# nygenome/Lancet2

Measured on AMD Instinct MI355X. Metric: microassembly windows/sec (whole node), higher is better.
Workload: dtype u8/i32 (f64 statistics)

## Files before the change

lancet2_amd/csrc/poa.hip:

```cpp
#include <algorithm>
#include <cstdio>
#include <cstdlib>
#include <vector>

#include "ma_internal.h"

namespace ma {

namespace {

constexpr int kT = 256;
constexpr u32 kSlowCap = 256;
constexpr u32 kMaxSeq = 32;
constexpr i32 kNegInf = static_cast<i32>(0x80000000u) + 1024;
constexpr i32 M_ = 0, N_ = -6, G_ = -6, E_ = -2, Q_ = -26, C_ = -1;

constexpr u32 kTierIn = 2;

constexpr u32 RI_FAST = 1u << 11;
constexpr u32 RI_SLOWTAB = 1u << 12;
constexpr u32 RI_STORE = 1u << 13;
constexpr u32 RI_LEAN = 1u << 14;
constexpr u32 RI_SLIDE = 1u << 15;
template <int PE>
// ... 38 lines not shown
  size_t frow_cells;
  u32 full_by_worker;
  u32 band_stride;
  u16* codes;
  i32* rows;
  i32* hlast;
  u32 split;
  u32 img_words;
  u8* img;
};

extern __shared__ __attribute__((aligned(16))) unsigned char ma_lds[];
template <class T>
struct LdsArr {
  u32 off;
  __device__ __forceinline__ T& operator[](u32 i) const { return *reinterpret_cast<T*>(&ma_lds[off + i * sizeof(T)]); }
};

struct WgState {
  u32 nn, nseq, nrank, overflow;
  i32 seq_first[kMaxSeq];
  u32 mode, V, L, cw, naln, nslow;
  u32 band, band_fail;
  u32 filled;
  i32 edge_max;
  i32 edge0;
  i32 best;
  u32 best_row;
  i32 ftot[2][4][2];
  i32 fbnd[2][4][4];
  u32 wsum[4];
  i32 red_v[4];
  u32 red_r[4];
  i32 begin, prev0, lastn;
  u32 nv;
  u32 x_done, x_a, x_ns;
  u32 win_overflow;
  u32 c_cur, h_cur, pending, done;
  u32 nvars, pool, var_overflow;
  i32 xa_active[kMaxSeq], xa_alt_of[kMaxSeq];
  u32 xa_hap_pos[kMaxSeq], xa_starts[kMaxSeq], xa_rawlen[kMaxSeq], xa_grp_rep[kMaxSeq], xa_glo[kMaxSeq], xa_ghi[kMaxSeq], xa_ordg[kMaxSeq],
      xa_rank_of_grp[kMaxSeq];
};
#define ST (*reinterpret_cast<WgState*>(ma_lds))
constexpr u32 kStBytes = (sizeof(WgState) + 15u) & ~15u;

template <int PE_>
struct GLT {
  static constexpr int pe = PE_;
  u32 pn;
  LdsArr<u8> nchar, nin, nout, nal;
  LdsArr<u16> in_tail, out_head, al, rank2node, node2rank;
  u32 lab32;
  u32 out_lab_off;
  __device__ __forceinline__ u32 lab(u32 i) const {
    return lab32 ? *reinterpret_cast<u32*>(&ma_lds[out_lab_off + 4u * i]) : static_cast<u32>(*reinterpret_cast<u16*>(&ma_lds[out_lab_off + 2u * i]));
  }
  __device__ __forceinline__ void lab_set(u32 i, u32 v) const {
    if (lab32) *reinterpret_cast<u32*>(&ma_lds[out_lab_off + 4u * i]) = v;
    else *reinterpret_cast<u16*>(&ma_lds[out_lab_off + 2u * i]) = static_cast<u16>(v);
  }
  __device__ __forceinline__ void lab_or(u32 i, u32 v) const { lab_set(i, lab(i) | v); }
  __device__ __forceinline__ u32 max_seq() const { return lab32 ? 32u : 16u; }
  LdsArr<u16> npos;
  LdsArr<u32> rowinfo;
  LdsArr<u16> rowslot, rowdepth, runhead, rowj0, slowpred, aln;
  u32 aln_cap;
  LdsArr<u16> cnode, cpos, ccur;
  LdsArr<u16> stack;
  LdsArr<u8> marks, ignored;
  u32 stack_cap;
  __device__ __forceinline__ u32 ubyte(const u8* p) const { return *p; }
  __device__ __forceinline__ u32 uword(const void* p) const { return *static_cast<const u32*>(p); }
};

__host__ __device__ inline size_t poa_lds_bytes(u32 pn, u32 ml, u32 lab32, u32 pe) {
  size_t const graph = size_t(10 + pe * (lab32 ? 10 : 8)) * pn;
  size_t const s_aln = size_t(12) * (pn + 2) + 2 * pe * kSlowCap + size_t(4) * (pn + ml + 2);
  size_t const s_topo = size_t(2 * pe + 2) * pn;
  return kStBytes + graph + (s_aln > s_topo ? s_aln : s_topo) + 16;
}

constexpr size_t kPoaLdsLimit = 160 * 1024 - 256;
inline u32 poa_node_capacity(u32 max_len, u32 lab32) {
  u32 pn = max_len + std::max<u32>(256, max_len / 4);
  pn = std::min<u32>((pn + 7) & ~7u, 65000);
  while (!lab32 && poa_lds_bytes(pn, max_len, lab32, 4) > 80 * 1024 && pn > max_len + 128) pn -= 8;
  while (poa_lds_bytes(pn, max_len, lab32, 4) > 159 * 1024 && pn > max_len + 32) pn -= 8;
  return pn;
}
inline u32 poa_node_capacity_max(u32 max_len, u32 lab32, u32 pe) {
  u32 const floor_pn = (max_len + 32 + 7) & ~7u;
  if (poa_lds_bytes(floor_pn, max_len, lab32, pe) > kPoaLdsLimit) return 0;
  u32 pn = floor_pn;
  while (pn + 8 <= 65000 && poa_lds_bytes(pn + 8, max_len, lab32, pe) <= kPoaLdsLimit) pn += 8;
  return pn;
}
inline u32 poa_retry_max_hap_len(u32 lab32, u32 pe) {
  u32 l = 4096;
  while (l > 16 && poa_node_capacity_max(l, lab32, pe) == 0) --l;
  return l;
}
inline u32 poa_max_hap_len(u32 lab32) {
  auto const scan = [](u32 lab) {
    u32 l = 4096;
    while (l > 16 && poa_lds_bytes(poa_node_capacity(l, lab), l, lab, 4) > kPoaLdsLimit) --l;
    return l;
  };
  static u32 const common = scan(0u), wide = scan(1u);
  return lab32 ? wide : common;
}

template <int PE>
__device__ __forceinline__ GLT<PE> poa_carve(u32 PN, u32 ML, u32 lab32) {
  GLT<PE> g;
  g.pn = PN;
  g.lab32 = lab32;
  u32 o = kStBytes;
  g.nchar.off = o;
  g.nin.off = o + PN;
  g.nout.off = o + 2 * PN;
  g.nal.off = o + 3 * PN;
  o += 4 * PN;
  g.in_tail.off = o;
  g.out_head.off = o + 2 * PE * PN;
  g.out_lab_off = o + 4 * PE * PN;
  g.al.off = o + (lab32 ? 8 : 6) * PE * PN;
  o += (lab32 ? 10 : 8) * PE * PN;
  g.rank2node.off = o;
  g.node2rank.off = o + 2 * PN;
  g.npos.off = o + 4 * PN;
  o += 6 * PN;
  u32 const S = o;
  g.rowinfo.off = S;
  g.rowslot.off = S + 4 * (PN + 2);
  g.rowdepth.off = S + 6 * (PN + 2);
  g.runhead.off = S + 8 * (PN + 2);
  g.rowj0.off = S + 10 * (PN + 2);
  g.slowpred.off = S + 12 * (PN + 2);
  g.aln.off = S + 12 * (PN + 2) + 2 * PE * kSlowCap;
  g.aln_cap = PN + ML + 2;
  g.cnode.off = S;
  g.cpos.off = S + 2 * (ML + 2);
  g.ccur.off = S + 4 * (ML + 2);
  g.stack.off = S;
  g.stack_cap = PE * PN;
  g.marks.off = S + 2 * PE * PN;
  g.ignored.off = S + (2 * PE + 1) * PN;
  return g;
}

__device__ __forceinline__ void lds_barrier() { asm volatile("s_waitcnt lgkmcnt(0)\n\ts_barrier" ::: "memory"); }

template <class G>
__device__ __forceinline__ i32 pg_add_node(G const& g, u8 ch, u32 pos) {
  if (ST.nn >= g.pn) {
    ST.overflow = 1;
    return 0;
  }
  u32 const id = ST.nn++;
  g.nchar[id] = ch;
  g.nin[id] = g.nout[id] = g.nal[id] = 0;
  g.npos[id] = static_cast<u16>(min(pos, 0xFFFFu));
  return static_cast<i32>(id);
}
template <class G>
__device__ __forceinline__ void pg_add_edge(G const& g, u32 tail, u32 head, u32 lab) {
  u32 const no = g.nout[tail];
  for (u32 x = 0; x < no; ++x)
    if (g.out_head[tail * G::pe + x] == head) {
      g.lab_or(tail * G::pe + x, lab);
      return;
    }
  u32 const ni = g.nin[head];
  if (no >= G::pe || ni >= G::pe) {
    atomicOr(&ST.overflow, kOvSlots);
    return;
  }
  g.out_head[tail * G::pe + no] = static_cast<u16>(head);
  g.lab_set(tail * G::pe + no, lab);
  g.nout[tail] = static_cast<u8>(no + 1);
  g.in_tail[head * G::pe + ni] = static_cast<u16>(tail);
  g.nin[head] = static_cast<u8>(ni + 1);
}
template <class G>
__device__ __forceinline__ i32 pg_add_sequence(G const& g, const u8* seq, u32 begin, u32 end) {
  if (begin >= end) return -1;
  i32 prev = -1;
  u32 const first = ST.nn;
  u32 const lab = 1u << ST.nseq;
  for (u32 i = begin; i < end; ++i) {
    i32 const cur = pg_add_node(g, seq[i], i);
    if (ST.overflow) return -1;
    if (prev >= 0) pg_add_edge(g, static_cast<u32>(prev), static_cast<u32>(cur), lab);
    prev = cur;
  }
  return static_cast<i32>(first);
}
template <class G>
__device__ __forceinline__ i32 pg_successor(G const& g, u32 node, u32 label) {
  for (int x = 0; x < g.nout[node]; ++x)
    if (g.lab(node * G::pe + x) & (1u << label)) return static_cast<i32>(g.out_head[node * G::pe + x]);
  return -1;
}
template <class G>
__device__ __forceinline__ void pg_toposort(G const& g, int lane) {
  u32 const nn = ST.nn;
  u32 nrank = 0, s = 0;
  u32 overflow = 0;
  LdsArr<u16> const stack = g.stack;
  while (s < nn && !overflow) {
    u32 const v = s + static_cast<u32>(lane);
    bool trivial = false, marked = false;
    if (v < nn) {
      marked = g.marks[v] != 0;
      if (!marked && g.nal[v] == 0) {
        u32 const ni = g.nin[v];
        bool ok = true;
        for (u32 x = 0; x < ni; ++x) ok = ok && g.in_tail[v * G::pe + x] < v;
        trivial = ok;
      }
    }
    unsigned long long const pm = __ballot(v < nn && (marked || trivial));
    u32 const run = pm == ~0ull ? 64u : static_cast<u32>(__builtin_ctzll(~pm));
    if (run > 0) {
      unsigned long long const keep = run == 64 ? ~0ull : ((1ull << run) - 1ull);
      unsigned long long const tm = __ballot(trivial) & keep;
      if (static_cast<u32>(lane) < run && trivial) {
        u32 const r = nrank + static_cast<u32>(__popcll(tm & ((1ull << lane) - 1ull)));
        g.rank2node[r] = static_cast<u16>(v);
        g.marks[v] = 2;
      }
      nrank += static_cast<u32>(__popcll(tm));
      s += run;
      continue;
    }
    if (lane == 0) {
      u32 sp = 0;
      stack[sp++] = static_cast<u16>(s);
      while (sp > 0) {
        u32 const cur = stack[sp - 1];
        bool valid = true;
        if (g.marks[cur] != 2) {
          for (int x = 0; x < g.nin[cur]; ++x) {
            u32 const t = g.in_tail[cur * G::pe + x];
            if (g.marks[t] != 2) {
              if (sp < g.stack_cap) stack[sp++] = static_cast<u16>(t); else overflow = 1;
              valid = false;
            }
          }
          if (!g.ignored[cur]) {
            for (int x = 0; x < g.nal[cur]; ++x) {
              u32 const an = g.al[cur * G::pe + x];
              if (g.marks[an] != 2) {
                if (sp < g.stack_cap) stack[sp++] = static_cast<u16>(an); else overflow = 1;
                g.ignored[an] = 1;
                valid = false;
              }
            }
          }
          if (valid) {
            g.marks[cur] = 2;
            if (!g.ignored[cur]) {
              g.rank2node[nrank++] = static_cast<u16>(cur);
              for (int x = 0; x < g.nal[cur]; ++x) g.rank2node[nrank++] = g.al[cur * G::pe + x];
            }
          } else {
            g.marks[cur] = 1;
          }
        }
        if (valid) sp--;
        if (overflow) break;
      }
    }
    nrank = __shfl(nrank, 0);
    overflow = __shfl(overflow, 0);
    s += 1;
  }
  if (lane == 0) {
    ST.nrank = nrank;
    if (overflow) ST.overflow = 1;
  }
}

__device__ __forceinline__ i32 classify_variant(const u8* r, u32 rl, const u8* a, u32 al) {
  u32 s = 0;
  while (s < rl && s < al && r[s] == a[s]) s++;
  if (s == rl && s == al) return -1;
  u32 e = 0;
  while (e < (rl - s) && e < (al - s) && r[rl - 1 - e] == a[al - 1 - e]) e++;
  u32 const rc = rl - s - e, ac = al - s - e;
  if (rc == 0 && ac > 0) return 1;
  if (rc > 0 && ac == 0) return 2;
  if (rc == 0 || ac == 0) return -1;
  if (rc != ac) return 4;
  return rc == 1 ? 0 : 3;
}
__device__ __forceinline__ i32 variant_length(const u8* r, u32 rl, const u8* a, u32 al, i32 t) {
  if (t == 0) return 1;
  i32 const R = static_cast<i32>(rl), A = static_cast<i32>(al);
  if (t == 1 || t == 2 || t == 4) return A - R;
  i32 s = 0;
  while (s < R && s < A && r[s] == a[s]) s++;
  i32 e = 0;
  while (e < (R - s) && e < (A - s) && r[R - 1 - e] == a[A - 1 - e]) e++;
  return A - s - e;
}
__device__ __forceinline__ int bytes_cmp(const u8* a, u32 al, const u8* b, u32 bl) {
  u32 const m = al < bl ? al : bl;
  for (u32 i = 0; i < m; ++i)
    if (a[i] != b[i]) return a[i] < b[i] ? -1 : 1;
  return al < bl ? -1 : (al > bl ? 1 : 0);
}

template <class G>
__device__ __forceinline__ u32 pred_row(G const& g, u32 i, u32 info, u32 x) {
  if (info & RI_FAST) return i - 1;
  if (info & RI_SLOWTAB) return g.slowpred[(G::pe <= 4 ? info >> 16 : (info >> 16) & 0xFFu) * G::pe + x];
  u32 const node = g.rank2node[i - 1];
  return static_cast<u32>(g.node2rank[g.in_tail[node * G::pe + x]]) + 1u;
// ... 1240 lines not shown
        rb[2 * static_cast<size_t>(w_stride) + c] = oo[c];
      }
      __threadfence_block();
    }
    if (L >= j0 && L < j0 + BW && static_cast<u32>(lane) == (L - j0) / CW) {
      u32 const cL = (L - j0) % CW;
      i32 v = hh[0];
#pragma unroll
      for (int c = 1; c < CW; ++c) v = (static_cast<u32>(c) == cL) ? hh[c] : v;
      hlast[i] = v;
    } else if (lane == 0 && !(L >= j0 && L < j0 + BW)) {
      hlast[i] = kNegInf;
    }
#pragma unroll
    for (int c = 0; c < CW; ++c) {
      H1[c] = hh[c];
      F1[c] = ff[c];
      O1[c] = oo[c];
    }
    __builtin_amdgcn_s_waitcnt(0);
  };

  u32 info = g.rowinfo[1];
  __builtin_amdgcn_s_waitcnt(0);
#ifdef MA_PROFILE
  unsigned long long t_lean = 0, t_gen = 0, n_gen = 0;
  unsigned long long const t_fill0 = __builtin_amdgcn_s_memtime();
#endif
  for (u32 i = 1; i <= V; ++i) {
    u32 const cur = info;
    if (i < V) info = g.rowinfo[i + 1];
#ifdef MA_PROFILE
    unsigned long long const q0 = __builtin_amdgcn_s_memtime();
#endif
    if (__builtin_expect((cur & RI_LEAN) != 0, 1)) {
      if (__builtin_expect((cur >> 16) == 0, 1)) row_lean(cur, std::false_type{});
      else row_lean(cur, std::true_type{});
    } else {
      row_gen(i, cur);
    }
#ifdef MA_PROFILE
    unsigned long long const q1 = __builtin_amdgcn_s_memtime();
    if (cur & RI_LEAN) t_lean += q1 - q0; else { t_gen += q1 - q0; n_gen++; }
#endif
    cp += BW;
  }
#ifdef MA_PROFILE
  if (lane == 0) {
    atomicAdd(&g_prof[8], t_lean);
    atomicAdd(&g_prof[9], t_gen);
    atomicAdd(&g_prof[10], n_gen);
    atomicAdd(&g_prof[11], 1ull);
    atomicAdd(&g_prof[12], static_cast<unsigned long long>(V));
    atomicAdd(&g_prof[13], __builtin_amdgcn_s_memtime() - t_fill0);
  }
#endif
  for (int off = 32; off > 0; off >>= 1) edge = max(edge, __shfl_xor(edge, off));
  if (lane == 0) *edge_out = edge;
}

struct EdgeVals {
  i32 h, f, e, o, q;
};
template <class G>
__device__ __forceinline__ EdgeVals edge_vals(G const& g, u32 i, u32 j) {
  EdgeVals v;
  if (i == 0 && j == 0) {
    v.h = v.f = v.e = v.o = v.q = 0;
  } else if (i == 0) {
    v.q = Q_ + static_cast<i32>(j - 1) * C_;
    v.e = G_ + static_cast<i32>(j - 1) * E_;
    v.h = max(v.q, v.e);
    v.f = v.o = kNegInf;
  } else {
    u32 const d = g.rowdepth[i];
    v.o = col0_o(d);
    v.f = col0_f(d);
    v.h = max(v.o, v.f);
    v.e = v.q = kNegInf;
  }
  return v;
}

template <class G>
__device__ __forceinline__ u32 poa_traceback(G const& g, const u16* codes16, size_t const plane, u32 cw, u32 V, u32 L, u32 best_row,
                             bool have_end, int lane, u32 bw) {
  const u8* const codes = reinterpret_cast<const u8*>(codes16);
  bool const band = bw != 0;
  u32 const nl = (L + cw - 1) / cw;
  bool off_band = false;
  auto code_at = [&](u32 i, u32 j) -> u32 {
    if (band) {
      u32 const j0 = g.rowj0[i];
      if (j < j0 || j >= j0 + bw) {
        off_band = true;
        return 2u;
      }
      size_t const at = static_cast<size_t>(i) * bw + (j - j0);
      u32 const a = codes[at];
      return (g.rowinfo[i] & RI_FAST) ? a : (a | (static_cast<u32>(codes[plane + at]) << 6));
    }
    size_t const at = static_cast<size_t>(i) * (nl * cw) + (j - 1);
    u32 const a = codes[at];
    return (g.rowinfo[i] & RI_FAST) ? a : (a | (static_cast<u32>(codes[plane + at]) << 6));
  };
  u32 naln = 0;
  bool overflow = false;
  auto push1 = [&](u32 node1, u32 pos1) {
    if (naln + 1 >= g.aln_cap) {
      overflow = true;
      return;
    }
    if (lane == 0) {
      g.aln[2 * naln] = static_cast<u16>(node1);
      g.aln[2 * naln + 1] = static_cast<u16>(pos1);
    }
    naln++;
  };
  u32 i = have_end ? best_row : 0u, j = have_end ? L : 0u;
  u32 prev_i = 0, prev_j = 0;
  while (!(i == 0 && j == 0) && !overflow && !__ballot(off_band)) {
    if (i >= 1 && j >= 1) {
      {
        u32 const k = static_cast<u32>(lane);
        bool ok = false;
        if (i >= k + 2 && j >= k + 1) ok = ((code_at(i - k, j - k) & 3u) == 0u) && (g.rowinfo[i - k] & RI_FAST);
        unsigned long long const m = __ballot(ok);
        u32 const run = m == ~0ull ? 64u : static_cast<u32>(__builtin_ctzll(~m));
        if (run > 0) {
          if (naln + run + 1 >= g.aln_cap) {
            overflow = true;
            break;
          }
          if (k < run) {
            g.aln[2 * (naln + k)] = static_cast<u16>(g.rank2node[i - k - 1] + 1u);
            g.aln[2 * (naln + k) + 1] = static_cast<u16>(j - k);
          }
          naln += run;
          i -= run;
          j -= run;
          prev_i = i;
          prev_j = j;
          continue;
        }
      }
      u32 const cd = code_at(i, j);
      u32 const info = g.rowinfo[i];
      u32 const np = ri_np<G::pe>(info);
      u32 const node = g.rank2node[i - 1];
      u32 const kind = cd & 3u;
      bool const ext = cd & 4u;
      constexpr u32 XB = kXB<G::pe>, XM = (1u << XB) - 1u;
      u32 const x = (cd >> 6) & XM;
      if (kind == 0) {
        prev_i = np ? pred_row(g, i, info, x) : 0u;
        prev_j = j - 1;
        push1(node + 1, j);
        i = prev_i;
        j = prev_j;
      } else if (kind == 1) {
        prev_i = np ? pred_row(g, i, info, x) : 0u;
        prev_j = j;
        push1(node + 1, 0);
        i = prev_i;
        if (ext) {
          while (!overflow && i >= 1) {
            {
              u32 const k = static_cast<u32>(lane);
              bool ok = false;
              if (i >= k + 2) ok = (code_at(i - k, j) & 16u) && (g.rowinfo[i - k] & RI_FAST);
              unsigned long long const m = __ballot(ok);
              u32 const run = m == ~0ull ? 64u : static_cast<u32>(__builtin_ctzll(~m));
              if (run > 0) {
                if (naln + run + 1 >= g.aln_cap) {
                  overflow = true;
                  break;
                }
                if (k < run) {
                  g.aln[2 * (naln + k)] = static_cast<u16>(g.rank2node[i - k - 1] + 1u);
                  g.aln[2 * (naln + k) + 1] = 0;
                }
                naln += run;
                i -= run;
                prev_i = i;
                continue;
              }
            }
            u32 const c2 = code_at(i, j);
            u32 const info2 = g.rowinfo[i];
            bool const us = c2 & 16u, uh = c2 & 32u;
            u32 const pi = (us || uh) ? pred_row(g, i, info2, (c2 >> (6 + XB)) & XM) : 0u;
            push1(g.rank2node[i - 1] + 1u, 0);
            prev_i = pi;
            i = pi;
            if (!us || i == 0) break;
          }
        }
      } else {
        prev_i = i;
        prev_j = j - 1;
        push1(0, j);
        j = prev_j;
        if (ext) {
          while (!overflow && j >= 1) {
            u32 const k = static_cast<u32>(lane);
            bool cont = false;
            if (j >= k + 1) cont = code_at(i, j - k) & 8u;
            unsigned long long const m = __ballot(cont);
            u32 const nc = m == ~0ull ? 64u : static_cast<u32>(__builtin_ctzll(~m));
            u32 const cnt = nc < 64u ? nc + 1u : 64u;
            if (naln + cnt + 1 >= g.aln_cap) {
              overflow = true;
              break;
            }
            if (k < cnt) {
              g.aln[2 * (naln + k)] = 0;
              g.aln[2 * (naln + k) + 1] = static_cast<u16>(j - k);
            }
            naln += cnt;
            j -= cnt;
            if (nc < 64u) break;
          }
        }
      }
      continue;
    }
    i32 const Hij = edge_vals(g, i, j).h;
    bool found = false, ext_left = false, ext_up = false;
    u32 const node = i ? g.rank2node[i - 1] : 0u;
    u32 const info = i ? g.rowinfo[i] : 0u;
    u32 const np = i ? (ri_np<G::pe>(info)) : 0u;
    if (i != 0) {
      for (u32 x = 0; x < (np ? np : 1u); ++x) {
        u32 const pi = np ? pred_row(g, i, info, x) : 0u;
        EdgeVals const pv = edge_vals(g, pi, j);
        bool ok = (ext_up |= (Hij == pv.f + E_));
        if (!ok) ok = Hij == pv.h + G_;
        if (!ok) ok = (ext_up |= (Hij == pv.o + C_));
        if (!ok) ok = Hij == pv.h + Q_;
        if (ok) {
          prev_i = pi;
          prev_j = j;
          found = true;
          break;
        }
      }
    }
    if (!found && j != 0) {
      EdgeVals const lv = edge_vals(g, i, j - 1);
      bool ok = (ext_left |= (Hij == lv.e + E_));
      if (!ok) ok = Hij == lv.h + G_;
      if (!ok) ok = (ext_left |= (Hij == lv.q + C_));
      if (!ok) ok = Hij == lv.h + Q_;
      if (ok) {
        prev_i = i;
        prev_j = j - 1;
        found = true;
      }
    }
    push1(i != prev_i ? node + 1 : 0u, j != prev_j ? j : 0u);
    i = prev_i;
    j = prev_j;
    if (ext_left) {
      while (!overflow) {
        push1(0, j);
        --j;
        bool const e_stop = edge_vals(g, i, j).e + E_ != edge_vals(g, i, j + 1).e;
        bool const q_stop = edge_vals(g, i, j).q + C_ != edge_vals(g, i, j + 1).q;
        if ((e_stop && q_stop) || j == 0) break;
      }
    } else if (ext_up) {
      while (!overflow && i >= 1) {
        bool stop = true;
        prev_i = 0;
        u32 const nd2 = g.rank2node[i - 1];
        u32 const info2 = g.rowinfo[i];
        u32 const np2 = ri_np<G::pe>(info2);
        EdgeVals const cv = edge_vals(g, i, j);
        for (u32 x = 0; x < np2; ++x) {
          u32 const pr = pred_row(g, i, info2, x);
          EdgeVals const pv = edge_vals(g, pr, j);
          if (cv.f == pv.f + E_ || cv.o == pv.o + C_) {
            prev_i = pr;
            stop = false;
            break;
          }
        }
        if (stop) {
          for (u32 x = 0; x < np2; ++x) {
            u32 const pr = pred_row(g, i, info2, x);
            i32 const hp2 = edge_vals(g, pr, j).h;
            if (cv.f == hp2 + G_ || cv.o == hp2 + Q_) {
              prev_i = pr;
              break;
            }
          }
        }
        push1(nd2 + 1u, 0);
        i = prev_i;
        if (stop || i == 0) break;
      }
    }
  }
  if (__ballot(off_band)) {
// ... 1345 lines not shown
  } else {
    MA_TRY_RC(launch_msa_pass(ctx, b, a, o, got[0], rounds, 0u, any_wide ? 1u : 0u, caps, cause));
    if (any_wide) MA_TRY_RC(launch_msa_pass(ctx, b, a, o, std::max(got[3], 16u), rounds, 1u, 2u, caps, cause));
  }
  if (!cause) return MA_OK;
  static RetryCaps const rcaps{{poa_retry_max_hap_len(0u, 8u), poa_retry_max_hap_len(1u, 8u), poa_retry_max_hap_len(0u, 4u), poa_retry_max_hap_len(1u, 4u)}};
  hipLaunchKernelGGL(k_poa_retry_select, dim3((n + 255) / 256), dim3(256), 0, ctx->stream, a, o.win_nvars, n, static_cast<u32>(P.max_haps),
                     static_cast<u32>(P.max_comps), cause, rcaps, all32 ? 1u : 0u, rctr);
  u32 marks[4] = {0, 0, 0, 0};
  MA_HIP(ctx, hipMemcpyAsync(marks, rctr, 16, hipMemcpyDeviceToHost, ctx->stream));
  MA_HIP(ctx, ma_stream_sync(ctx));
  ctx->poa_retry_counts[0] = marks[0];
  ctx->poa_retry_counts[1] = marks[1];
  if (marks[0] + marks[1] == 0) return MA_OK;
  u32 mx[5] = {0, 0, 0, 0, 0};
  MA_HIP(ctx, hipMemcpyAsync(mx, rctr + 4, 20, hipMemcpyDeviceToHost, ctx->stream));
  MA_HIP(ctx, ma_stream_sync(ctx));
  u32 const rrounds = std::max<u32>(1u, mx[4] + 1u);
  for (u32 k = 0; k < 4; ++k)
    if (mx[k]) MA_TRY_RC(launch_msa_pass(ctx, b, a, o, mx[k], rrounds, k & 1u, 3u + k, caps, cause));
  hipLaunchKernelGGL(k_poa_retry_count, dim3((n + 255) / 256), dim3(256), 0, ctx->stream, a, n, static_cast<const u8*>(cause), rctr);
  MA_HIP(ctx, hipMemcpyAsync(marks, rctr, 16, hipMemcpyDeviceToHost, ctx->stream));
  MA_HIP(ctx, ma_stream_sync(ctx));
  ctx->poa_retry_counts[2] = marks[2];
  ctx->poa_retry_counts[3] = marks[3];
  return MA_OK;
}
static int launch_msa_pass(ma_ctx* ctx, const DBatch& b, const ma_asm_out_t& a, const ma_var_out_t& o, u32 max_len, u32 rounds,
                           u32 const lab32, u32 const pass, const u32 (&len_caps)[3], u8* const cause) {
  int const n = b.n_windows;
  ma_params_t const& P = ctx->prm;
  PoaWs ws{};
  MA_TRY_RC(ma_dev_stats(ctx, &ws.dstats));
  ws.lab32 = lab32;
  ws.pass = pass;
  ws.cause = cause;
  bool const retry = pass >= 3;
  u32 const pe = (pass == 3 || pass == 4) ? 8u : 4u;
  ws.len_cap16 = len_caps[0];
  ws.len_cap32 = len_caps[1];
  ws.len_all32 = len_caps[2];
  max_len = std::max<u32>(max_len, 16);
  ws.max_l = max_len;
  u32 const pn = retry ? poa_node_capacity_max(max_len, lab32, pe) : poa_node_capacity(max_len, lab32);
  size_t const lds = poa_lds_bytes(pn, max_len, lab32, pe);
  if (pn == 0 || lds > kPoaLdsLimit) {
    ma_set_err(ctx, "ma_msa_batch: haplotypes too long for the LDS-resident POA graph");
    return MA_ERR_PARAM;
  }
  ws.pn = pn;
  ws.w_stride = (max_len + 7) & ~7u;
  ws.row_slots = pn / 2;
  int const band_mode = getenv("MA_POA_BAND") ? atoi(getenv("MA_POA_BAND")) : 2;
  ws.use_band = (band_mode != 0 && band_mode != 3) ? 1u : 0u;
  ws.split = band_mode >= 2 ? 1u : 0u;
  ws.no_direct = getenv("MA_POA_NO_DIRECT") ? 1u : 0u;
  ws.raw_cap = getenv("MA_POA_RAW_CAP") ? static_cast<u32>(atoi(getenv("MA_POA_RAW_CAP"))) : 0u;
  ws.lean = (getenv("MA_POA_LEAN") && atoi(getenv("MA_POA_LEAN")) == 0) ? 0u : 1u;
  {
    int const t0 = getenv("MA_POA_TIER0") ? atoi(getenv("MA_POA_TIER0")) : static_cast<int>(kTierIn);
    ws.tier0 = (t0 == 1 || t0 == 2) ? static_cast<u32>(t0) : 4u;
  }
  u32 const min_pending = getenv("MA_POA_MIN_PENDING") ? static_cast<u32>(atoi(getenv("MA_POA_MIN_PENDING"))) : 256u;
  bool const verbose = getenv("MA_VERBOSE") != nullptr;
  ws.img_words = static_cast<u32>((lds + 3) / 4);
  ws.band_stride = 256;
  ws.code_cells = (static_cast<size_t>(pn + 2) * 256 + 7) & ~size_t(7);
  if (ws.code_cells * 2 < static_cast<size_t>(P.max_haps) * (2 * max_len + 8) + 64)
    ws.code_cells = (static_cast<size_t>(P.max_haps) * (2 * max_len + 8) / 2 + 64 + 7) & ~size_t(7);
  ws.row_cells = static_cast<size_t>(ws.row_slots) * 3 * ws.band_stride;
  ws.fcode_cells = (static_cast<size_t>(pn + 2) * (max_len + 16) + 7) & ~size_t(7);
  ws.frow_cells = static_cast<size_t>(ws.row_slots) * 3 * ws.w_stride;
  size_t const full_bytes = ((ws.fcode_cells * 2 + 255) & ~size_t(255)) + ((ws.frow_cells * 4 + 255) & ~size_t(255));

  size_t const img_bytes = ws.split ? ((static_cast<size_t>(ws.img_words) * 4 + 255) & ~size_t(255)) : 0;
  ws.img_words = static_cast<u32>(ws.split ? img_bytes / 4 : ws.img_words);
  bool const sched = !retry && ws.split && ws.lean && !(getenv("MA_POA_SCHED") && atoi(getenv("MA_POA_SCHED")) == 0);
  ws.full_by_worker = sched ? 1u : 0u;
  int n_cu = 256;
  {
    hipDeviceProp_t prop;
    if (hipGetDeviceProperties(&prop, ctx->device) == hipSuccess && prop.multiProcessorCount > 0) n_cu = prop.multiProcessorCount;
  }
  int wgs_per_cu = lds > 80 * 1024 ? 1 : 2;
  if (const char* e = getenv("MA_POA_WGS_PER_CU")) wgs_per_cu = std::max(1, std::min(wgs_per_cu, atoi(e)));
  size_t const per_window = ws.code_cells * 2 + ws.row_cells * 4 + (static_cast<size_t>(pn) + 8) * 4 + img_bytes + (sched ? 0 : full_bytes);
  (void)rounds;
  size_t budget = stage_budget(0.30, ctx->ws_build.cap, size_t(24) << 30, ctx->hbm_share);
  if (const char* e = getenv("MA_WS_GB")) budget = static_cast<size_t>(atoi(e)) << 30;
  size_t const max_workers = sched ? std::max<size_t>(1, std::min<size_t>(std::min<size_t>(n, static_cast<size_t>(n_cu) * wgs_per_cu),
                                                                        budget / 2 / full_bytes)) : 0;
  size_t const fixed_bytes = max_workers * full_bytes;
  int const chunk = static_cast<int>(std::max<size_t>(1, std::min<size_t>(n, (budget > fixed_bytes ? budget - fixed_bytes : 0) / per_window)));
  u32 qcap = 64;
  while (qcap < static_cast<u32>(chunk)) qcap <<= 1;
  MA_HIP(ctx, ctx->ws_build.reserve(per_window * static_cast<size_t>(chunk) + fixed_bytes + 16384 + 3 * sizeof(u32) * qcap * kPoaDoms +
                                  sizeof(PoaSched) + sizeof(u32) * qcap));
  u32 const xcd_local = (getenv("MA_POA_XCD") && atoi(getenv("MA_POA_XCD")) == 0) ? 0u : 1u;
  if (getenv("MA_VERBOSE"))
    fprintf(stderr, "[microasm] msa: %d windows, %.2f MB/window + %zu full-fill areas of %.2f MB, budget %.1f GB -> chunks of %d (pn %u, max_len %u, lds %zu)\n",
            n, per_window / 1048576.0, max_workers, full_bytes / 1048576.0, budget / 1073741824.0, chunk, pn, max_len, lds);
  auto kern = lab32 ? (max_len <= 1024 ? k_msa<4, true, 4> : (max_len <= 2048 ? k_msa<8, true, 4> : k_msa<16, true, 4>))
                    : (max_len <= 1024 ? k_msa<4, false, 4> : (max_len <= 2048 ? k_msa<8, false, 4> : k_msa<16, false, 4>));
  if (pe == 8)
    kern = lab32 ? (max_len <= 1024 ? k_msa<4, true, 8> : k_msa<8, true, 8>) : (max_len <= 1024 ? k_msa<4, false, 8> : k_msa<8, false, 8>);
  MA_HIP(ctx, hipFuncSetAttribute(reinterpret_cast<const void*>(kern), hipFuncAttributeMaxDynamicSharedMemorySize,
                                  static_cast<int>(lds)));
  auto pkern = lab32 ? (max_len <= 1024 ? k_poa<4, true> : (max_len <= 2048 ? k_poa<8, true> : k_poa<16, true>))
                     : (max_len <= 1024 ? k_poa<4, false> : (max_len <= 2048 ? k_poa<8, false> : k_poa<16, false>));
  if (sched)
    MA_HIP(ctx, hipFuncSetAttribute(reinterpret_cast<const void*>(pkern), hipFuncAttributeMaxDynamicSharedMemorySize,
                                    static_cast<int>(lds)));
  for (int win0 = 0; win0 < n; win0 += chunk) {
    int const nwin = std::min(chunk, n - win0);
    char* base = static_cast<char*>(ctx->ws_build.p);
    size_t const csz = (static_cast<size_t>(nwin) * ws.code_cells * 2 + 255) & ~size_t(255);
    size_t const rsz = (static_cast<size_t>(nwin) * ws.row_cells * 4 + 255) & ~size_t(255);
    ws.codes = reinterpret_cast<u16*>(base);
    ws.rows = reinterpret_cast<i32*>(base + csz);
    ws.hlast = reinterpret_cast<i32*>(base + csz + rsz);
    size_t const hsz = (static_cast<size_t>(nwin) * (pn + 8) * 4 + 255) & ~size_t(255);
    ws.img = reinterpret_cast<u8*>(base + csz + rsz + hsz);
    size_t const n_full = sched ? max_workers : static_cast<size_t>(nwin);
    size_t const isz = (static_cast<size_t>(nwin) * img_bytes + 255) & ~size_t(255);
    size_t const fcsz = (n_full * ws.fcode_cells * 2 + 255) & ~size_t(255);
    size_t const frsz = (n_full * ws.frow_cells * 4 + 255) & ~size_t(255);
    ws.fcodes = reinterpret_cast<u16*>(base + csz + rsz + hsz + isz);
    ws.frows = reinterpret_cast<i32*>(base + csz + rsz + hsz + isz + fcsz);
    {
      u32* ctr = reinterpret_cast<u32*>(base + csz + rsz + hsz + isz + fcsz + frsz);
      ctr = reinterpret_cast<u32*>((reinterpret_cast<uintptr_t>(ctr) + 255) & ~uintptr_t(255));
      ws.pending_ctr = ctr;
      ws.tier_stats = verbose ? ctr + 8 : nullptr;
      if (!sched) MA_HIP(ctx, hipMemsetAsync(ctr, 0, 64, ctx->stream));
    }
    MsaArgs args{b, a, o, ws, P, win0, 0u, 0u};
    if (sched) {
      char* qb = reinterpret_cast<char*>(ws.pending_ctr) + 256;
      PoaSched* const S = reinterpret_cast<PoaSched*>(qb);
      u32* const fq = reinterpret_cast<u32*>(qb + sizeof(PoaSched));
      u32* const gq = fq + static_cast<size_t>(qcap) * kPoaDoms;
      u32* const hq = gq + static_cast<size_t>(qcap) * kPoaDoms;
      u32 const grid = static_cast<u32>(std::min<size_t>(static_cast<size_t>(nwin), max_workers));
      MA_HIP(ctx, hipMemsetAsync(ws.pending_ctr, 0, 256 + sizeof(PoaSched), ctx->stream));
      MA_HIP(ctx, hipMemsetAsync(fq, 0xFF, 3 * sizeof(u32) * qcap * kPoaDoms, ctx->stream));
      u32* const order = hq + static_cast<size_t>(qcap) * kPoaDoms;
      hipLaunchKernelGGL(k_poa_order, dim3(1), dim3(1024), 0, ctx->stream, args, order, static_cast<u32>(nwin));
      ctx->tic("k_poa");
      hipLaunchKernelGGL(pkern, dim3(grid), dim3(kT), lds, ctx->stream, args, S, fq, gq, hq, qcap, static_cast<u32>(nwin), xcd_local, kPoaMinFills,
                         static_cast<const u32*>(order));
      ctx->toc();
      if (verbose) {
        PoaSched hs;
        MA_HIP(ctx, hipMemcpyAsync(&hs, S, sizeof(hs), hipMemcpyDeviceToHost, ctx->stream));
        MA_HIP(ctx, ma_stream_sync(ctx));
        fprintf(stderr, "[microasm] k_poa: %u workgroups, %d windows; per XCD (workgroups / windows started):", grid, nwin);
        for (u32 x = 0; x < kPoaDoms; ++x)
          if (hs.dom[x].seen) fprintf(stderr, " %u: %u / %u", x, hs.dom[x].seen, hs.dom[x].started);
        fprintf(stderr, "\n");
      }
    } else if (!ws.split) {
      args.finish = 1;
      ctx->tic("k_msa");
      hipLaunchKernelGGL(kern, dim3(nwin), dim3(kT), lds, ctx->stream, args);
      ctx->toc();
    } else {
      size_t const band_lds = kStBytes + 16 + 256;
      u32 const max_rounds = 2u * rounds + 2u;
      for (u32 r = 0;; ++r) {
        args.round = r;
        args.finish = 0;
        ctx->tic("k_msa");
        hipLaunchKernelGGL(kern, dim3(nwin), dim3(kT), lds, ctx->stream, args);
        ctx->toc();
        u32 pend2[2] = {0, 0};
        MA_HIP(ctx, hipMemcpyAsync(pend2, ws.pending_ctr, 8, hipMemcpyDeviceToHost, ctx->stream));
        MA_HIP(ctx, hipMemsetAsync(ws.pending_ctr, 0, 8, ctx->stream));
        MA_HIP(ctx, ma_stream_sync(ctx));
        u32 const pending = pend2[0], pending_retry = pend2[1];
        if (pending == 0) break;
        if ((pending < min_pending && pending_retry == 0) || r + 1 >= max_rounds) {
          args.round = r + 1;
          args.finish = 1;
          ctx->tic("k_msa");
          hipLaunchKernelGGL(kern, dim3(nwin), dim3(kT), lds, ctx->stream, args);
          ctx->toc();
          break;
        }
        ctx->tic("k_msa_band");
        auto band = [&](auto kfn) { hipLaunchKernelGGL(kfn, dim3(nwin), dim3(64), band_lds, ctx->stream, args); };
        if (pe == 8) {
          if (ws.lean) band(k_msa_band<true, 8>);
          else band(k_msa_band<false, 8>);
        } else if (ws.lean) {
          band(k_msa_band<true, 4>);
        } else {
          band(k_msa_band<false, 4>);
        }
        ctx->toc();
      }
    }
    if (verbose) {
      u32 tsx[8];
      MA_HIP(ctx, hipMemcpyAsync(tsx, ws.tier_stats, 32, hipMemcpyDeviceToHost, ctx->stream));
      MA_HIP(ctx, ma_stream_sync(ctx));
      fprintf(stderr, "[microasm] msa tiers: fills 64/128/256 = %u/%u/%u, failed certificates = %u/%u/%u\n", tsx[0], tsx[1],
              tsx[2], tsx[4], tsx[5], tsx[6]);
    }
    MA_HIP(ctx, hipGetLastError());
  }
  return MA_OK;
}

}
```

Before: 305,800.

## Widen toposort and traceback wave scans to multi-chunk lookahead and fix occupancy sizing

The wavefront scans in the topological sort and in the traceback (diagonal, vertical and horizontal runs) now prefetch four 64-lane chunks per iteration instead of one. Toposort also treats a node as trivial when its predecessors are already marked, and it places simple alignment rings in parallel before falling back to the serial DFS. The worker count per CU now accounts for static LDS and is capped by the occupancy API, and the POA kernel attribute is set earlier. This cuts loop iterations and serial fallbacks on long runs, at the cost of extra speculative LDS/global reads, more registers and more complex control flow.

New measurement: 308,800 (median of 6 runs). No clear change (+1.0%).

```diff
diff --git a/lancet2_amd/csrc/poa.hip b/lancet2_amd/csrc/poa.hip
--- a/lancet2_amd/csrc/poa.hip
+++ b/lancet2_amd/csrc/poa.hip
@@ -144,10 +144,11 @@
 }
 
 constexpr size_t kPoaLdsLimit = 160 * 1024 - 256;
+constexpr size_t kPoaStaticLds = 32;
 inline u32 poa_node_capacity(u32 max_len, u32 lab32) {
   u32 pn = max_len + std::max<u32>(256, max_len / 4);
   pn = std::min<u32>((pn + 7) & ~7u, 65000);
-  while (!lab32 && poa_lds_bytes(pn, max_len, lab32, 4) > 80 * 1024 && pn > max_len + 128) pn -= 8;
+  while (!lab32 && poa_lds_bytes(pn, max_len, lab32, 4) > 80 * 1024 - kPoaStaticLds && pn > max_len + 128) pn -= 8;
   while (poa_lds_bytes(pn, max_len, lab32, 4) > 159 * 1024 && pn > max_len + 32) pn -= 8;
   return pn;
 }
@@ -265,6 +266,7 @@
     if (g.lab(node * G::pe + x) & (1u << label)) return static_cast<i32>(g.out_head[node * G::pe + x]);
   return -1;
 }
+constexpr u32 kTopoChunks = 4;
 template <class G>
 __device__ __forceinline__ void pg_toposort(G const& g, int lane) {
   u32 const nn = ST.nn;
@@ -272,32 +274,78 @@
   u32 overflow = 0;
   LdsArr<u16> const stack = g.stack;
   while (s < nn && !overflow) {
-    u32 const v = s + static_cast<u32>(lane);
-    bool trivial = false, marked = false;
-    if (v < nn) {
-      marked = g.marks[v] != 0;
-      if (!marked && g.nal[v] == 0) {
-        u32 const ni = g.nin[v];
+    bool trivial[kTopoChunks], marked[kTopoChunks];
+#pragma unroll
+    for (u32 c = 0; c < kTopoChunks; ++c) {
+      u32 const v = s + 64u * c + static_cast<u32>(lane);
+      trivial[c] = marked[c] = false;
+      if (v < nn) {
+        u32 const mk = g.marks[v], na = g.nal[v], ni = g.nin[v];
         bool ok = true;
-        for (u32 x = 0; x < ni; ++x) ok = ok && g.in_tail[v * G::pe + x] < v;
-        trivial = ok;
-      }
-    }
-    unsigned long long const pm = __ballot(v < nn && (marked || trivial));
-    u32 const run = pm == ~0ull ? 64u : static_cast<u32>(__builtin_ctzll(~pm));
-    if (run > 0) {
-      unsigned long long const keep = run == 64 ? ~0ull : ((1ull << run) - 1ull);
-      unsigned long long const tm = __ballot(trivial) & keep;
-      if (static_cast<u32>(lane) < run && trivial) {
-        u32 const r = nrank + static_cast<u32>(__popcll(tm & ((1ull << lane) - 1ull)));
-        g.rank2node[r] = static_cast<u16>(v);
-        g.marks[v] = 2;
-      }
-      nrank += static_cast<u32>(__popcll(tm));
-      s += run;
-      continue;
-    }
-    if (lane == 0) {
+#pragma unroll
+        for (u32 x = 0; x < static_cast<u32>(G::pe); ++x) {
+          u32 const t = g.in_tail[v * G::pe + x];
+          ok = ok && (t < v || x >= ni || g.marks[x < ni ? t : v] == 2);
+        }
+        marked[c] = mk != 0;
+        trivial[c] = mk == 0 && na == 0 && ok;
+      }
+    }
+    bool all_full = true;
+#pragma unroll
+    for (u32 c = 0; c < kTopoChunks; ++c) {
+      u32 const v = s + static_cast<u32>(lane);
+      unsigned long long const pm = __ballot(v < nn && (marked[c] || trivial[c]));
+      u32 const run = pm == ~0ull ? 64u : static_cast<u32>(__builtin_ctzll(~pm));
+      if (run > 0) {
+        unsigned long long const keep = run == 64 ? ~0ull : ((1ull << run) - 1ull);
+        unsigned long long const tm = __ballot(trivial[c]) & keep;
+        if (static_cast<u32>(lane) < run && trivial[c]) {
+          u32 const r = nrank + static_cast<u32>(__popcll(tm & ((1ull << lane) - 1ull)));
+          g.rank2node[r] = static_cast<u16>(v);
+          g.marks[v] = 2;
+        }
+        nrank += static_cast<u32>(__popcll(tm));
+        s += run;
+      }
+      if (run < 64u) {
+        all_full = false;
+        break;
+      }
+    }
+    if (all_full || s >= nn) continue;
+    bool ring = false;
+    {
+      u32 const na = g.nal[s];
+      if (na > 0) {
+        bool good = true;
+        u32 node = s;
+        if (static_cast<u32>(lane) < na) node = g.al[s * G::pe + static_cast<u32>(lane)];
+        if (static_cast<u32>(lane) < na || lane == G::pe) {
+          u32 const ni = g.nin[node];
+          good = lane == G::pe ? g.ignored[s] == 0 : g.marks[node] == 0;
+#pragma unroll
+          for (u32 x = 0; x < static_cast<u32>(G::pe); ++x) {
+            u32 const t = g.in_tail[node * G::pe + x];
+            good = good && (x >= ni || g.marks[x < ni ? t : node] == 2);
+          }
+        }
+        ring = __ballot(!good) == 0ull;
+        if (ring) {
+          if (static_cast<u32>(lane) < na) {
+            g.marks[node] = 2;
+            g.ignored[node] = 1;
+            g.rank2node[nrank + 1 + static_cast<u32>(lane)] = static_cast<u16>(node);
+          }
+          if (lane == G::pe) {
+            g.marks[s] = 2;
+            g.rank2node[nrank] = static_cast<u16>(s);
+          }
+          nrank += 1 + na;
+        }
+      }
+    }
+    if (!ring && lane == 0) {
       u32 sp = 0;
       stack[sp++] = static_cast<u16>(s);
       while (sp > 0) {
@@ -1704,6 +1752,7 @@
   return v;
 }
 
+constexpr u32 kTbChunks = 4;
 template <class G>
 __device__ __forceinline__ u32 poa_traceback(G const& g, const u16* codes16, size_t const plane, u32 cw, u32 V, u32 L, u32 best_row,
                              bool have_end, int lane, u32 bw) {
@@ -1726,6 +1775,19 @@
     u32 const a = codes[at];
     return (g.rowinfo[i] & RI_FAST) ? a : (a | (static_cast<u32>(codes[plane + at]) << 6));
   };
+  constexpr u32 kPeekOff = 1u << 30, kPeekNone = 1u << 31;
+  auto peek = [&](u32 i, u32 j, bool with_b) -> u32 {
+    size_t at;
+    if (band) {
+      u32 const j0 = g.rowj0[i];
+      if (j < j0 || j >= j0 + bw) return kPeekOff;
+      at = static_cast<size_t>(i) * bw + (j - j0);
+    } else {
+      at = static_cast<size_t>(i) * (nl * cw) + (j - 1);
+    }
+    u32 const a = codes[at];
+    return (with_b && !(g.rowinfo[i] & RI_FAST)) ? (a | (static_cast<u32>(codes[plane + at]) << 6)) : a;
+  };
   u32 naln = 0;
   bool overflow = false;
   auto push1 = [&](u32 node1, u32 pos1) {
@@ -1743,30 +1805,65 @@
   u32 prev_i = 0, prev_j = 0;
   while (!(i == 0 && j == 0) && !overflow && !__ballot(off_band)) {
     if (i >= 1 && j >= 1) {
+      u32 stop_code = kPeekNone;
       {
         u32 const k = static_cast<u32>(lane);
-        bool ok = false;
-        if (i >= k + 2 && j >= k + 1) ok = ((code_at(i - k, j - k) & 3u) == 0u) && (g.rowinfo[i - k] & RI_FAST);
-        unsigned long long const m = __ballot(ok);
-        u32 const run = m == ~0ull ? 64u : static_cast<u32>(__builtin_ctzll(~m));
-        if (run > 0) {
-          if (naln + run + 1 >= g.aln_cap) {
-            overflow = true;
+        u32 av[kTbChunks];
+        bool fs[kTbChunks];
+#pragma unroll
+        for (u32 c = 0; c < kTbChunks; ++c) {
+          u32 const kk = 64u * c + k;
+          av[c] = kPeekNone;
+          fs[c] = false;
+          if (i >= kk + 2 && j >= kk + 1) {
+            av[c] = peek(i - kk, j - kk, true);
+            fs[c] = g.rowinfo[i - kk] & RI_FAST;
+          }
+        }
+        bool again = false;
+#pragma unroll
+        for (u32 c = 0; c < kTbChunks; ++c) {
+          if (av[c] == kPeekOff) off_band = true;
+          unsigned long long const m = __ballot((av[c] & (kPeekOff | kPeekNone | 3u)) == 0u && fs[c]);
+          u32 const run = m == ~0ull ? 64u : static_cast<u32>(__builtin_ctzll(~m));
+          if (run > 0) {
+            if (naln + run + 1 >= g.aln_cap) {
+              overflow = true;
+              again = true;
+              break;
+            }
+            if (k < run) {
+              g.aln[2 * (naln + k)] = static_cast<u16>(g.rank2node[i - k - 1] + 1u);
+              g.aln[2 * (naln + k) + 1] = static_cast<u16>(j - k);
+            }
+            naln += run;
+            i -= run;
+            j -= run;
+            prev_i = i;
+            prev_j = j;
+          }
+          if (__ballot(off_band)) {
+            again = true;
             break;
           }
-          if (k < run) {
-            g.aln[2 * (naln + k)] = static_cast<u16>(g.rank2node[i - k - 1] + 1u);
-            g.aln[2 * (naln + k) + 1] = static_cast<u16>(j - k);
-          }
-          naln += run;
-          i -= run;
-          j -= run;
-          prev_i = i;
-          prev_j = j;
-          continue;
-        }
-      }
-      u32 const cd = code_at(i, j);
+          if (run == 64u) {
+            again = c + 1 == kTbChunks;
+            continue;
+          }
+          stop_code = __shfl(av[c], static_cast<int>(run));
+          if (run > 0) {
+            if (c + 1 < kTbChunks) {
+              if (k < run && av[c + 1 < kTbChunks ? c + 1 : c] == kPeekOff) off_band = true;
+              again = __ballot(off_band) != 0;
+            } else {
+              again = true;
+            }
+          }
+          break;
+        }
+        if (again || j == 0) continue;
+      }
+      u32 const cd = (stop_code & (kPeekOff | kPeekNone)) ? code_at(i, j) : stop_code;
       u32 const info = g.rowinfo[i];
       u32 const np = ri_np<G::pe>(info);
       u32 const node = g.rank2node[i - 1];
@@ -1789,24 +1886,42 @@
           while (!overflow && i >= 1) {
             {
               u32 const k = static_cast<u32>(lane);
-              bool ok = false;
-              if (i >= k + 2) ok = (code_at(i - k, j) & 16u) && (g.rowinfo[i - k] & RI_FAST);
-              unsigned long long const m = __ballot(ok);
-              u32 const run = m == ~0ull ? 64u : static_cast<u32>(__builtin_ctzll(~m));
-              if (run > 0) {
-                if (naln + run + 1 >= g.aln_cap) {
-                  overflow = true;
-                  break;
+              u32 av[kTbChunks];
+              bool fs[kTbChunks];
+#pragma unroll
+              for (u32 c = 0; c < kTbChunks; ++c) {
+                u32 const kk = 64u * c + k;
+                av[c] = kPeekNone;
+                fs[c] = false;
+                if (i >= kk + 2) {
+                  av[c] = peek(i - kk, j, false);
+                  fs[c] = g.rowinfo[i - kk] & RI_FAST;
                 }
-                if (k < run) {
-                  g.aln[2 * (naln + k)] = static_cast<u16>(g.rank2node[i - k - 1] + 1u);
-                  g.aln[2 * (naln + k) + 1] = 0;
+              }
+              bool moved = false;
+#pragma unroll
+              for (u32 c = 0; c < kTbChunks; ++c) {
+                if (av[c] == kPeekOff) off_band = true;
+                unsigned long long const m = __ballot((av[c] & (kPeekOff | kPeekNone)) == 0u && (av[c] & 16u) && fs[c]);
+                u32 const run = m == ~0ull ? 64u : static_cast<u32>(__builtin_ctzll(~m));
+                if (run > 0) {
+                  if (naln + run + 1 >= g.aln_cap) {
+                    overflow = true;
+                    break;
+                  }
+                  if (k < run) {
+                    g.aln[2 * (naln + k)] = static_cast<u16>(g.rank2node[i - k - 1] + 1u);
+                    g.aln[2 * (naln + k) + 1] = 0;
+                  }
+                  naln += run;
+                  i -= run;
+                  prev_i = i;
+                  moved = true;
                 }
-                naln += run;
-                i -= run;
-                prev_i = i;
-                continue;
+                if (run < 64u) break;
               }
+              if (overflow) break;
+              if (moved) continue;
             }
             u32 const c2 = code_at(i, j);
             u32 const info2 = g.rowinfo[i];
@@ -1826,22 +1941,36 @@
         if (ext) {
           while (!overflow && j >= 1) {
             u32 const k = static_cast<u32>(lane);
-            bool cont = false;
-            if (j >= k + 1) cont = code_at(i, j - k) & 8u;
-            unsigned long long const m = __ballot(cont);
-            u32 const nc = m == ~0ull ? 64u : static_cast<u32>(__builtin_ctzll(~m));
-            u32 const cnt = nc < 64u ? nc + 1u : 64u;
-            if (naln + cnt + 1 >= g.aln_cap) {
-              overflow = true;
-              break;
+            u32 av[kTbChunks];
+#pragma unroll
+            for (u32 c = 0; c < kTbChunks; ++c) {
+              u32 const kk = 64u * c + k;
+              av[c] = j >= kk + 1 ? peek(i, j - kk, false) : kPeekNone;
             }
-            if (k < cnt) {
-              g.aln[2 * (naln + k)] = 0;
-              g.aln[2 * (naln + k) + 1] = static_cast<u16>(j - k);
+            bool ended = false;
+#pragma unroll
+            for (u32 c = 0; c < kTbChunks; ++c) {
+              if (j < 1) break;
+              if (av[c] == kPeekOff) off_band = true;
+              unsigned long long const m = __ballot((av[c] & (kPeekOff | kPeekNone)) == 0u && (av[c] & 8u));
+              u32 const nc = m == ~0ull ? 64u : static_cast<u32>(__builtin_ctzll(~m));
+              u32 const cnt = nc < 64u ? nc + 1u : 64u;
+              if (naln + cnt + 1 >= g.aln_cap) {
+                overflow = true;
+                break;
+              }
+              if (k < cnt) {
+                g.aln[2 * (naln + k)] = 0;
+                g.aln[2 * (naln + k) + 1] = static_cast<u16>(j - k);
+              }
+              naln += cnt;
+              j -= cnt;
+              if (nc < 64u) {
+                ended = true;
+                break;
+              }
             }
-            naln += cnt;
-            j -= cnt;
-            if (nc < 64u) break;
+            if (overflow || ended) break;
           }
         }
       }
@@ -3353,7 +3482,18 @@
     hipDeviceProp_t prop;
     if (hipGetDeviceProperties(&prop, ctx->device) == hipSuccess && prop.multiProcessorCount > 0) n_cu = prop.multiProcessorCount;
   }
-  int wgs_per_cu = lds > 80 * 1024 ? 1 : 2;
+  auto pkern = lab32 ? (max_len <= 1024 ? k_poa<4, true> : (max_len <= 2048 ? k_poa<8, true> : k_poa<16, true>))
+                     : (max_len <= 1024 ? k_poa<4, false> : (max_len <= 2048 ? k_poa<8, false> : k_poa<16, false>));
+  int wgs_per_cu = lds + kPoaStaticLds > 80 * 1024 ? 1 : 2;
+  if (sched) {
+    MA_HIP(ctx, hipFuncSetAttribute(reinterpret_cast<const void*>(pkern), hipFuncAttributeMaxDynamicSharedMemorySize,
+                                    static_cast<int>(lds)));
+    int resident = 0;
+    if (hipOccupancyMaxActiveBlocksPerMultiprocessor(&resident, reinterpret_cast<const void*>(pkern), kT, lds) == hipSuccess && resident >= 1)
+      wgs_per_cu = std::min(wgs_per_cu, resident);
+    else
+      (void)hipGetLastError();
+  }
   if (const char* e = getenv("MA_POA_WGS_PER_CU")) wgs_per_cu = std::max(1, std::min(wgs_per_cu, atoi(e)));
   size_t const per_window = ws.code_cells * 2 + ws.row_cells * 4 + (static_cast<size_t>(pn) + 8) * 4 + img_bytes + (sched ? 0 : full_bytes);
   (void)rounds;
@@ -3377,11 +3517,6 @@
     kern = lab32 ? (max_len <= 1024 ? k_msa<4, true, 8> : k_msa<8, true, 8>) : (max_len <= 1024 ? k_msa<4, false, 8> : k_msa<8, false, 8>);
   MA_HIP(ctx, hipFuncSetAttribute(reinterpret_cast<const void*>(kern), hipFuncAttributeMaxDynamicSharedMemorySize,
                                   static_cast<int>(lds)));
-  auto pkern = lab32 ? (max_len <= 1024 ? k_poa<4, true> : (max_len <= 2048 ? k_poa<8, true> : k_poa<16, true>))
-                     : (max_len <= 1024 ? k_poa<4, false> : (max_len <= 2048 ? k_poa<8, false> : k_poa<16, false>));
-  if (sched)
-    MA_HIP(ctx, hipFuncSetAttribute(reinterpret_cast<const void*>(pkern), hipFuncAttributeMaxDynamicSharedMemorySize,
-                                    static_cast<int>(lds)));
   for (int win0 = 0; win0 < n; win0 += chunk) {
     int const nwin = std::min(chunk, n - win0);
     char* base = static_cast<char*>(ctx->ws_build.p);
@@ -3425,7 +3560,8 @@
         PoaSched hs;
         MA_HIP(ctx, hipMemcpyAsync(&hs, S, sizeof(hs), hipMemcpyDeviceToHost, ctx->stream));
         MA_HIP(ctx, ma_stream_sync(ctx));
-        fprintf(stderr, "[microasm] k_poa: %u workgroups, %d windows; per XCD (workgroups / windows started):", grid, nwin);
+        fprintf(stderr, "[microasm] k_poa: %u workgroups (%d per CU, pn %u, lds %zu), %d windows; per XCD (workgroups / windows started):", grid,
+                wgs_per_cu, pn, lds, nwin);
         for (u32 x = 0; x < kPoaDoms; ++x)
           if (hs.dom[x].seen) fprintf(stderr, " %u: %u / %u", x, hs.dom[x].seen, hs.dom[x].started);
         fprintf(stderr, "\n");
```
